# AlanLiangC/SPSNet

Measured on NVIDIA B200. Metric: IA-SSD SA-backbone scenes/s (16k pts), higher is better.
Workload: dtype fp16 operands / fp32 accumulate (split-fp16 hi+lo for K <= 64 chains and all Conv1d GEMMs); fp32 + int32 sampling

## Files before the change

spsnet_b200/csrc/pw_mma.cu:

```cuda
#include "mma_ptx.cuh"

namespace spsk {

constexpr int PW_ROWS = 128;
constexpr int PW_THREADS = 192;
constexpr int PW_TILE_BYTES = 16384;
constexpr int pw_smem(int stages, bool split) { return 256 + stages * (split ? 4 : 2) * PW_TILE_BYTES; }

struct PwArgs {
    int rows, k, ldx, n, npad, n_kc, relu;
    int split, xlo;
    int o16lo;
    const __half *x;
    const __half *wtiles;
    const float *bias;
    float *out_cm; int m, c_total, co_off;
    __half *out16; int ld16, n16;
    float *out_pm; int ldpm;
    unsigned int *ovf; unsigned int ovf_bit;
};

template <int PW_STAGES, int PW_LAG, bool SPLIT>
__global__ void __launch_bounds__(PW_THREADS, (PW_STAGES <= 3 && !SPLIT) ? 2 : 1)
pw_mma_kernel(const PwArgs a) {
    constexpr int STAGE_BYTES = (SPLIT ? 4 : 2) * PW_TILE_BYTES;
    extern __shared__ __align__(128) uint8_t smem[];
    uint64_t *bars = reinterpret_cast<uint64_t *>(smem);
    uint32_t *tmem_slot = reinterpret_cast<uint32_t *>(smem + 192);
    uint8_t *stage0 = smem + 256;
    const uint32_t bar0 = smem_u32(bars);
    auto FULL = [&](int s) { return bar0 + 8u * s; };
    auto EMPTY = [&](int s) { return bar0 + 8u * (PW_STAGES + s); };
    const uint32_t ACC_FULL = bar0 + 8u * (2 * PW_STAGES);
    auto XS = [&](int s) { return stage0 + (size_t)s * STAGE_BYTES; };
    auto WS = [&](int s) { return stage0 + (size_t)s * STAGE_BYTES + (SPLIT ? 2 : 1) * PW_TILE_BYTES; };

    const int tid = threadIdx.x, warp = tid >> 5, lane = tid & 31;
    const int tile = blockIdx.x, cc = blockIdx.y;
    const int ncols = min(128, a.npad - cc * 128);

    if (tid == 0) {
        for (int s = 0; s < PW_STAGES; ++s) { mbar_init(FULL(s), 128 + 1); mbar_init(EMPTY(s), 1); }
        mbar_init(ACC_FULL, 1);
        mbar_init_fence();
    }
    if (warp == 5) tmem_alloc(smem_u32(tmem_slot), 128);
    tc_fence_before();
    __syncthreads();
    tc_fence_after();
    const uint32_t tmem_base = *tmem_slot;

    if (warp == 4) {
        const bool leader = elect_one();
        for (int kc = 0; kc < a.n_kc; ++kc) {
            const int s = kc % PW_STAGES;
            const uint32_t ph = (kc / PW_STAGES) & 1u;
            mbar_wait(EMPTY(s), ph ^ 1u);
            if (leader) {
                constexpr uint32_t WB = (SPLIT ? 2 : 1) * PW_TILE_BYTES;
                mbar_expect_tx(FULL(s), WB);
                bulk_g2s(smem_u32(WS(s)), a.wtiles + (size_t)(cc * a.n_kc + kc) * (WB / 2), WB, FULL(s));
            }
            __syncwarp();
        }
    } else if (warp == 5) {
        const bool leader = elect_one();
        const uint32_t idesc = umma_idesc(128, ncols);
        for (int kc = 0; kc < a.n_kc; ++kc) {
            const int s = kc % PW_STAGES;
            const uint32_t ph = (kc / PW_STAGES) & 1u;
            mbar_wait(FULL(s), ph);
            tc_fence_after();
            const uint32_t xb = smem_u32(XS(s)), wb = smem_u32(WS(s));
            const int nk16 = min(4, (a.k - kc * 64) / 16);
            if (leader) {
                for (int j = 0; j < nk16; ++j) {
                    const uint64_t xh = umma_desc(xb + (uint32_t)j * 256u, 128u, 1024u), wh = umma_desc(wb + (uint32_t)j * 256u, 128u, 1024u);
                    umma_f16(tmem_base, xh, wh, idesc, (kc | j) ? 1u : 0u);
                    if (SPLIT) {
                        umma_f16(tmem_base, umma_desc(xb + PW_TILE_BYTES + (uint32_t)j * 256u, 128u, 1024u), wh, idesc, 1u);
                        umma_f16(tmem_base, xh, umma_desc(wb + PW_TILE_BYTES + (uint32_t)j * 256u, 128u, 1024u), idesc, 1u);
                    }
                }
                umma_commit(EMPTY(s));
                if (kc == a.n_kc - 1) umma_commit(ACC_FULL);
            }
            __syncwarp();
        }
    } else {
        const int r8 = lane & 7, gq = lane >> 3;
        for (int kc = 0; kc < a.n_kc; ++kc) {
            const int s = kc % PW_STAGES;
            const uint32_t ph = (kc / PW_STAGES) & 1u;
            mbar_wait(EMPTY(s), ph ^ 1u);
            const uint32_t xs = smem_u32(XS(s));
            const int ng = min(8, (a.k - kc * 64) / 8);
#pragma unroll
            for (int it = 0; it < 4; ++it) {
                const int r = warp * 32 + it * 8 + r8;
                const long long row = (long long)tile * PW_ROWS + r;
                const bool ok = row < a.rows;
                const __half *src = a.x + (size_t)(ok ? row : 0) * a.ldx;
#pragma unroll
                for (int j = 0; j < 2; ++j) {
                    const int g = gq + 4 * j;
                    if (g < ng) {
                        const int col = kc * 64 + g * 8;
                        const uint32_t dst = xs + (uint32_t)(r >> 3) * 1024u + (uint32_t)g * 128u + (uint32_t)(r & 7) * 16u;
                        cp_async16(dst, src + col, ok ? 16u : 0u);
                        if (SPLIT) cp_async16(dst + PW_TILE_BYTES, src + a.xlo + col, ok ? 16u : 0u);
                    }
                }
            }
            cp_async_commit();
            if (kc >= PW_LAG) {
                cp_async_wait<PW_LAG>();
                fence_proxy_async();
                mbar_arrive(FULL((kc - PW_LAG) % PW_STAGES));
            }
        }
        cp_async_wait<0>();
        fence_proxy_async();
        for (int kc = max(a.n_kc - PW_LAG, 0); kc < a.n_kc; ++kc) mbar_arrive(FULL(kc % PW_STAGES));

        mbar_wait(ACC_FULL, 0u);
        tc_fence_after();
        const int r = tid;
        const long long row = (long long)tile * PW_ROWS + r;
        const bool ok = row < a.rows;
        const uint32_t taddr = tmem_base + ((uint32_t)(warp * 32) << 16);
        const int ch0 = cc * 128;
        long long bb = 0;
        int p = 0;
        if (a.out_cm && ok) { bb = row / a.m; p = (int)(row - bb * a.m); }
        float mx16 = 0.f;
        for (int c0 = 0; c0 < ncols; c0 += 16) {
            float v[16];
            __syncwarp();
            tmem_ld16(taddr + (uint32_t)c0, v);
            const float4 *b4 = reinterpret_cast<const float4 *>(a.bias + ch0 + c0);
#pragma unroll
            for (int i = 0; i < 4; ++i) {
                const float4 bv = __ldg(b4 + i);
                v[4 * i] += bv.x; v[4 * i + 1] += bv.y; v[4 * i + 2] += bv.z; v[4 * i + 3] += bv.w;
            }
            if (a.relu) {
#pragma unroll
                for (int i = 0; i < 16; ++i) v[i] = fmaxf(v[i], 0.f);
            }
            if (ok && a.out_cm) {
                float *o = a.out_cm + ((size_t)bb * a.c_total + a.co_off + ch0 + c0) * a.m + p;
#pragma unroll
                for (int i = 0; i < 16; ++i)
                    if (ch0 + c0 + i < a.n) o[(size_t)i * a.m] = v[i];
            }
            if (ok && a.out16) {
                __half *o = a.out16 + (size_t)row * a.ld16 + ch0 + c0;
#pragma unroll
                for (int q = 0; q < 2; ++q)
                    if (ch0 + c0 + 8 * q < a.n16) {
                        uint32_t h[4], l[4];
#pragma unroll
                        for (int i = 0; i < 4; ++i) {
                            mx16 = fmaxf(fmaxf(mx16, fabsf(v[8 * q + 2 * i])), fabsf(v[8 * q + 2 * i + 1]));
                            const __half2 hh = __floats2half2_rn(v[8 * q + 2 * i], v[8 * q + 2 * i + 1]);
                            const float2 hf = __half22float2(hh);
                            h[i] = *reinterpret_cast<const uint32_t *>(&hh);
                            l[i] = pack_h2(v[8 * q + 2 * i] - hf.x, v[8 * q + 2 * i + 1] - hf.y);
                        }
                        *reinterpret_cast<uint4 *>(o + 8 * q) = make_uint4(h[0], h[1], h[2], h[3]);
                        if (a.o16lo > 0) *reinterpret_cast<uint4 *>(o + a.o16lo + 8 * q) = make_uint4(l[0], l[1], l[2], l[3]);
                    }
            }
            if (ok && a.out_pm) {
                float *o = a.out_pm + (size_t)row * a.ldpm + ch0 + c0;
#pragma unroll
                for (int i = 0; i < 16; ++i)
                    if (ch0 + c0 + i < a.n) o[i] = v[i];
            }
        }
        if (mx16 > FP16_MAX && a.ovf) atomicOr(a.ovf, a.ovf_bit);
    }

    tc_fence_before();
    __syncthreads();
    if (warp == 5) {
        tc_fence_after();
        tmem_dealloc(tmem_base, 128);
    }
}

}

extern "C" int spsk_pw_mma_forward(const spsk_pw_desc *d, spsk_stream_t stream) {
    using namespace spsk;
    SPSK_REQUIRE(d, SPSK_ERR_INVALID_ARG, "pw_mma: null descriptor");
    SPSK_REQUIRE(d->rows >= 0 && d->n >= 1 && d->k >= 16 && d->k % 16 == 0 && d->ldx >= d->k && d->ldx % 8 == 0, SPSK_ERR_INVALID_ARG,
                 "pw_mma: bad sizes rows=%d k=%d ldx=%d n=%d (k multiple of 16, ldx multiple of 8)", d->rows, d->k, d->ldx, d->n);
    if (d->rows == 0) return SPSK_OK;
    SPSK_REQUIRE(d->x && d->wtiles && d->bias, SPSK_ERR_INVALID_ARG, "pw_mma: null input pointer");
    SPSK_REQUIRE(d->out_cm || d->out16 || d->out_pm, SPSK_ERR_INVALID_ARG, "pw_mma: no output requested");
    SPSK_REQUIRE((reinterpret_cast<uintptr_t>(d->x) & 15) == 0 && (reinterpret_cast<uintptr_t>(d->wtiles) & 15) == 0, SPSK_ERR_INVALID_ARG,
                 "pw_mma: x / wtiles must be 16-byte aligned");
    PwArgs a{};
    a.rows = d->rows; a.k = d->k; a.ldx = d->ldx; a.n = d->n; a.relu = d->relu ? 1 : 0;
    a.npad = (d->n + 15) / 16 * 16;
    a.split = d->split ? 1 : 0;
    a.xlo = d->xlo;
    a.n_kc = (d->k + 63) / 64;
    if (a.split)
        SPSK_REQUIRE(d->xlo >= d->k && d->xlo % 8 == 0 && d->xlo + d->k <= d->ldx, SPSK_ERR_INVALID_ARG,
                     "pw_mma: split input needs the lo part at a column xlo >= k, multiple of 8, inside ldx");
    a.x = reinterpret_cast<const __half *>(d->x);
    a.wtiles = reinterpret_cast<const __half *>(d->wtiles);
    a.bias = d->bias;
    a.out_cm = d->out_cm; a.m = d->m; a.c_total = d->c_total; a.co_off = d->co_off;
    if (a.out_cm)
        SPSK_REQUIRE(d->m >= 1 && d->rows % d->m == 0 && d->co_off >= 0 && d->co_off + d->n <= d->c_total, SPSK_ERR_INVALID_ARG,
                     "pw_mma: channel-major output needs rows %% m == 0 and a channel window inside c_total");
    a.out16 = reinterpret_cast<__half *>(d->out16); a.ld16 = d->ld16; a.n16 = d->n16; a.o16lo = d->o16lo;
    if (a.out16 && d->o16lo)
        SPSK_REQUIRE(d->o16lo >= d->n16 && d->o16lo % 8 == 0 && d->o16lo + d->n16 <= d->ld16, SPSK_ERR_INVALID_ARG,
                     "pw_mma: residual columns [o16lo, o16lo + n16) must follow the values inside ld16");
    if (a.out16)
        SPSK_REQUIRE(d->ld16 % 8 == 0 && d->n16 % 8 == 0 && d->n16 >= d->n && d->n16 <= d->ld16 &&
                         (reinterpret_cast<uintptr_t>(d->out16) & 15) == 0,
                     SPSK_ERR_INVALID_ARG, "pw_mma: fp16 output needs ld16, n16 multiples of 8, n <= n16 <= ld16, 16-byte alignment");
    a.out_pm = d->out_pm; a.ldpm = d->ldpm;
    a.ovf = fp16_overflow_word();
    a.ovf_bit = 1u << (d->ovf_tag & 31);
    if (a.out_pm) SPSK_REQUIRE(d->ldpm >= d->n, SPSK_ERR_INVALID_ARG, "pw_mma: ldpm < n");
    const bool deep = !a.split && a.n_kc >= 12;
    static SmemAttrOnce attr_s, attr_d, attr_x;
    if (a.split) {
        if (int rc = attr_x.ensure(reinterpret_cast<const void *>(pw_mma_kernel<3, 2, true>), pw_smem(3, true), "pw_mma_kernel<3,2,split>")) return rc;
    } else if (deep) {
        if (int rc = attr_d.ensure(reinterpret_cast<const void *>(pw_mma_kernel<6, 4, false>), pw_smem(6, false), "pw_mma_kernel<6,4>")) return rc;
    } else {
        if (int rc = attr_s.ensure(reinterpret_cast<const void *>(pw_mma_kernel<3, 2, false>), pw_smem(3, false), "pw_mma_kernel<3,2>")) return rc;
    }
    const int ncover = a.out16 ? max(a.npad, a.n16) : a.npad;
    a.npad = (ncover + 15) / 16 * 16;
    dim3 grid((unsigned)((d->rows + PW_ROWS - 1) / PW_ROWS), (unsigned)((a.npad + 127) / 128));
    if (a.split) pw_mma_kernel<3, 2, true><<<grid, PW_THREADS, pw_smem(3, true), as_stream(stream)>>>(a);
    else if (deep) pw_mma_kernel<6, 4, false><<<grid, PW_THREADS, pw_smem(6, false), as_stream(stream)>>>(a);
    else pw_mma_kernel<3, 2, false><<<grid, PW_THREADS, pw_smem(3, false), as_stream(stream)>>>(a);
    SPSK_LAUNCH_CHECK("pw_mma_kernel");
    return SPSK_OK;
}
```

Baseline: 12010.

## Make pointwise MMA kernel persistent with double-buffered TMEM and column-tile grouping

Result: no change. 12010, median of 6 (-0.0%).

```diff
diff --git a/spsnet_b200/csrc/pw_mma.cu b/spsnet_b200/csrc/pw_mma.cu
--- a/spsnet_b200/csrc/pw_mma.cu
+++ b/spsnet_b200/csrc/pw_mma.cu
@@ -3,14 +3,22 @@
 namespace spsk {
 
 constexpr int PW_ROWS = 128;
-constexpr int PW_THREADS = 192;
+constexpr int PW_THREADS = 320;
 constexpr int PW_TILE_BYTES = 16384;
-constexpr int pw_smem(int stages, bool split) { return 256 + stages * (split ? 4 : 2) * PW_TILE_BYTES; }
+constexpr int PW_HDR = 256;
+constexpr int PW_MAX_STAGES = 8;
+constexpr int PW_SMEM_TWO = 113 * 1024;
+constexpr int PW_SMEM_MAX = 227 * 1024;
 
 struct PwArgs {
     int rows, k, ldx, n, npad, n_kc, relu;
     int split, xlo;
     int o16lo;
+    int stages, lag;
+    int nct, gtiles, ngroups;
+    int items;
+    int wbytes;
+    int acc_cols;
     const __half *x;
     const __half *wtiles;
     const float *bias;
@@ -20,173 +28,236 @@
     unsigned int *ovf; unsigned int ovf_bit;
 };
 
-template <int PW_STAGES, int PW_LAG, bool SPLIT>
-__global__ void __launch_bounds__(PW_THREADS, (PW_STAGES <= 3 && !SPLIT) ? 2 : 1)
+__device__ __forceinline__ void cp_async_wait_n(int n) {
+    switch (n) {
+        case 1: cp_async_wait<1>(); break;
+        case 2: cp_async_wait<2>(); break;
+        case 3: cp_async_wait<3>(); break;
+        default: cp_async_wait<4>(); break;
+    }
+}
+
+__device__ __forceinline__ void pw_wait(uint32_t bar, uint32_t parity) {
+#pragma unroll 1
+    for (uint32_t spin = 0; spin < (1u << 27); ++spin) {
+        uint32_t done;
+        asm volatile(
+            "{\n\t.reg .pred p;\n\t"
+            "mbarrier.test_wait.parity.shared::cta.b64 p, [%1], %2;\n\t"
+            "selp.b32 %0, 1, 0, p;\n\t}"
+            : "=r"(done)
+            : "r"(bar), "r"(parity)
+            : "memory");
+        if (done) return;
+    }
+    __trap();
+}
+
+template <bool SPLIT>
+__global__ void __launch_bounds__(PW_THREADS, 2)
 pw_mma_kernel(const PwArgs a) {
-    constexpr int STAGE_BYTES = (SPLIT ? 4 : 2) * PW_TILE_BYTES;
+    constexpr uint32_t XBYTES = (SPLIT ? 2 : 1) * PW_TILE_BYTES;
+    constexpr uint32_t WTBYTES = (SPLIT ? 2 : 1) * PW_TILE_BYTES;
     extern __shared__ __align__(128) uint8_t smem[];
-    uint64_t *bars = reinterpret_cast<uint64_t *>(smem);
-    uint32_t *tmem_slot = reinterpret_cast<uint32_t *>(smem + 192);
-    uint8_t *stage0 = smem + 256;
-    const uint32_t bar0 = smem_u32(bars);
+    uint32_t *tmem_slot = reinterpret_cast<uint32_t *>(smem + PW_HDR - 16);
+    const int S = a.stages;
+    const uint32_t stage_bytes = XBYTES + (uint32_t)a.wbytes;
+    const uint32_t bar0 = smem_u32(smem), ring = bar0 + PW_HDR;
     auto FULL = [&](int s) { return bar0 + 8u * s; };
-    auto EMPTY = [&](int s) { return bar0 + 8u * (PW_STAGES + s); };
-    const uint32_t ACC_FULL = bar0 + 8u * (2 * PW_STAGES);
-    auto XS = [&](int s) { return stage0 + (size_t)s * STAGE_BYTES; };
-    auto WS = [&](int s) { return stage0 + (size_t)s * STAGE_BYTES + (SPLIT ? 2 : 1) * PW_TILE_BYTES; };
+    auto EMPTY = [&](int s) { return bar0 + 8u * (S + s); };
+    auto ACC_FULL = [&](uint32_t b) { return bar0 + 8u * (2 * S + b); };
+    auto ACC_EMPTY = [&](uint32_t b) { return bar0 + 8u * (2 * S + 2 + b); };
+    auto XS = [&](int s) { return ring + (uint32_t)s * stage_bytes; };
+    auto WS = [&](int s) { return ring + (uint32_t)s * stage_bytes + XBYTES; };
+    auto NCOLS = [&](int cc) { return min(128, a.npad - cc * 128); };
 
     const int tid = threadIdx.x, warp = tid >> 5, lane = tid & 31;
-    const int tile = blockIdx.x, cc = blockIdx.y;
-    const int ncols = min(128, a.npad - cc * 128);
 
     if (tid == 0) {
-        for (int s = 0; s < PW_STAGES; ++s) { mbar_init(FULL(s), 128 + 1); mbar_init(EMPTY(s), 1); }
-        mbar_init(ACC_FULL, 1);
+        for (int s = 0; s < S; ++s) { mbar_init(FULL(s), 128 + 1); mbar_init(EMPTY(s), 1); }
+        for (uint32_t b = 0; b < 2; ++b) { mbar_init(ACC_FULL(b), 1); mbar_init(ACC_EMPTY(b), 128); }
         mbar_init_fence();
     }
-    if (warp == 5) tmem_alloc(smem_u32(tmem_slot), 128);
+    if (warp == 9) tmem_alloc(smem_u32(tmem_slot), 2u * (uint32_t)a.acc_cols);
     tc_fence_before();
     __syncthreads();
     tc_fence_after();
     const uint32_t tmem_base = *tmem_slot;
 
-    if (warp == 4) {
+    if (warp == 8) {
         const bool leader = elect_one();
-        for (int kc = 0; kc < a.n_kc; ++kc) {
-            const int s = kc % PW_STAGES;
-            const uint32_t ph = (kc / PW_STAGES) & 1u;
-            mbar_wait(EMPTY(s), ph ^ 1u);
-            if (leader) {
-                constexpr uint32_t WB = (SPLIT ? 2 : 1) * PW_TILE_BYTES;
-                mbar_expect_tx(FULL(s), WB);
-                bulk_g2s(smem_u32(WS(s)), a.wtiles + (size_t)(cc * a.n_kc + kc) * (WB / 2), WB, FULL(s));
+        uint32_t q = 0;
+        for (int item = blockIdx.x; item < a.items; item += gridDim.x) {
+            const int cc0 = (item % a.ngroups) * a.gtiles, nt = min(a.gtiles, a.nct - cc0);
+            for (int kc = 0; kc < a.n_kc; ++kc, ++q) {
+                const int s = (int)(q % (uint32_t)S);
+                pw_wait(EMPTY(s), ((q / (uint32_t)S) & 1u) ^ 1u);
+                if (leader) {
+                    mbar_expect_tx(FULL(s), (uint32_t)(min(a.npad - cc0 * 128, nt * 128) * 128 * (SPLIT ? 2 : 1)));
+                    for (int t = 0; t < nt; ++t) {
+                        const int cc = cc0 + t;
+                        const uint32_t wb = (uint32_t)NCOLS(cc) * 128u;
+                        const __half *src = a.wtiles + (size_t)(cc * a.n_kc + kc) * (WTBYTES / 2);
+                        const uint32_t dst = WS(s) + (uint32_t)t * WTBYTES;
+                        if (SPLIT && wb < (uint32_t)PW_TILE_BYTES) {
+                            bulk_g2s(dst, src, wb, FULL(s));
+                            bulk_g2s(dst + wb, src + PW_TILE_BYTES / 2, wb, FULL(s));
+                        } else {
+                            bulk_g2s(dst, src, SPLIT ? 2u * wb : wb, FULL(s));
+                        }
+                    }
+                }
+                __syncwarp();
             }
-            __syncwarp();
         }
-    } else if (warp == 5) {
+    } else if (warp == 9) {
         const bool leader = elect_one();
-        const uint32_t idesc = umma_idesc(128, ncols);
-        for (int kc = 0; kc < a.n_kc; ++kc) {
-            const int s = kc % PW_STAGES;
-            const uint32_t ph = (kc / PW_STAGES) & 1u;
-            mbar_wait(FULL(s), ph);
+        uint32_t q = 0, i = 0;
+        for (int item = blockIdx.x; item < a.items; item += gridDim.x, ++i) {
+            const int cc0 = (item % a.ngroups) * a.gtiles, nt = min(a.gtiles, a.nct - cc0);
+            const uint32_t acc = i & 1u;
+            pw_wait(ACC_EMPTY(acc), ((i >> 1) & 1u) ^ 1u);
             tc_fence_after();
-            const uint32_t xb = smem_u32(XS(s)), wb = smem_u32(WS(s));
-            const int nk16 = min(4, (a.k - kc * 64) / 16);
-            if (leader) {
-                for (int j = 0; j < nk16; ++j) {
-                    const uint64_t xh = umma_desc(xb + (uint32_t)j * 256u, 128u, 1024u), wh = umma_desc(wb + (uint32_t)j * 256u, 128u, 1024u);
-                    umma_f16(tmem_base, xh, wh, idesc, (kc | j) ? 1u : 0u);
-                    if (SPLIT) {
-                        umma_f16(tmem_base, umma_desc(xb + PW_TILE_BYTES + (uint32_t)j * 256u, 128u, 1024u), wh, idesc, 1u);
-                        umma_f16(tmem_base, xh, umma_desc(wb + PW_TILE_BYTES + (uint32_t)j * 256u, 128u, 1024u), idesc, 1u);
-                    }
-                }
-                umma_commit(EMPTY(s));
-                if (kc == a.n_kc - 1) umma_commit(ACC_FULL);
+            const uint32_t d0 = tmem_base + acc * (uint32_t)a.acc_cols;
+            for (int kc = 0; kc < a.n_kc; ++kc, ++q) {
+                const int s = (int)(q % (uint32_t)S);
+                pw_wait(FULL(s), (q / (uint32_t)S) & 1u);
+                tc_fence_after();
+                const uint32_t xb = XS(s), wb = WS(s);
+                const int nk16 = min(4, (a.k - kc * 64) / 16);
+                if (leader) {
+                    for (int j = 0; j < nk16; ++j) {
+                        const uint64_t xh = umma_desc(xb + (uint32_t)j * 256u, 128u, 1024u);
+                        for (int t = 0; t < nt; ++t) {
+                            const int nc = NCOLS(cc0 + t);
+                            const uint32_t idesc = umma_idesc(128, nc), d = d0 + (uint32_t)t * 128u;
+                            const uint32_t wt = wb + (uint32_t)t * WTBYTES + (uint32_t)j * 256u;
+                            const uint64_t wh = umma_desc(wt, 128u, 1024u);
+                            umma_f16(d, xh, wh, idesc, (kc | j) ? 1u : 0u);
+                            if (SPLIT) {
+                                umma_f16(d, umma_desc(xb + PW_TILE_BYTES + (uint32_t)j * 256u, 128u, 1024u), wh, idesc, 1u);
+                                umma_f16(d, xh, umma_desc(wt + (uint32_t)nc * 128u, 128u, 1024u), idesc, 1u);
+                            }
+                        }
+                    }
+                    umma_commit(EMPTY(s));
+                    if (kc == a.n_kc - 1) umma_commit(ACC_FULL(acc));
+                }
+                __syncwarp();
             }
-            __syncwarp();
         }
-    } else {
-        const int r8 = lane & 7, gq = lane >> 3;
-        for (int kc = 0; kc < a.n_kc; ++kc) {
-            const int s = kc % PW_STAGES;
-            const uint32_t ph = (kc / PW_STAGES) & 1u;
-            mbar_wait(EMPTY(s), ph ^ 1u);
-            const uint32_t xs = smem_u32(XS(s));
-            const int ng = min(8, (a.k - kc * 64) / 8);
-#pragma unroll
-            for (int it = 0; it < 4; ++it) {
-                const int r = warp * 32 + it * 8 + r8;
-                const long long row = (long long)tile * PW_ROWS + r;
-                const bool ok = row < a.rows;
-                const __half *src = a.x + (size_t)(ok ? row : 0) * a.ldx;
-#pragma unroll
-                for (int j = 0; j < 2; ++j) {
-                    const int g = gq + 4 * j;
-                    if (g < ng) {
-                        const int col = kc * 64 + g * 8;
-                        const uint32_t dst = xs + (uint32_t)(r >> 3) * 1024u + (uint32_t)g * 128u + (uint32_t)(r & 7) * 16u;
-                        cp_async16(dst, src + col, ok ? 16u : 0u);
-                        if (SPLIT) cp_async16(dst + PW_TILE_BYTES, src + a.xlo + col, ok ? 16u : 0u);
-                    }
-                }
-            }
-            cp_async_commit();
-            if (kc >= PW_LAG) {
-                cp_async_wait<PW_LAG>();
-                fence_proxy_async();
-                mbar_arrive(FULL((kc - PW_LAG) % PW_STAGES));
+    } else if (warp >= 4) {
+        const int r8 = lane & 7, gq = lane >> 3, lw = warp - 4;
+        uint32_t q = 0;
+        for (int item = blockIdx.x; item < a.items; item += gridDim.x) {
+            const long long row0 = (long long)(item / a.ngroups) * PW_ROWS;
+            for (int kc = 0; kc < a.n_kc; ++kc, ++q) {
+                const int s = (int)(q % (uint32_t)S);
+                pw_wait(EMPTY(s), ((q / (uint32_t)S) & 1u) ^ 1u);
+                const uint32_t xs = XS(s);
+                const int ng = min(8, (a.k - kc * 64) / 8);
+#pragma unroll
+                for (int it = 0; it < 4; ++it) {
+                    const int r = lw * 32 + it * 8 + r8;
+                    const long long row = row0 + r;
+                    const bool ok = row < a.rows;
+                    const __half *src = a.x + (size_t)(ok ? row : 0) * a.ldx;
+#pragma unroll
+                    for (int j = 0; j < 2; ++j) {
+                        const int g = gq + 4 * j;
+                        if (g < ng) {
+                            const int col = kc * 64 + g * 8;
+                            const uint32_t dst = xs + (uint32_t)(r >> 3) * 1024u + (uint32_t)g * 128u + (uint32_t)(r & 7) * 16u;
+                            cp_async16(dst, src + col, ok ? 16u : 0u);
+                            if (SPLIT) cp_async16(dst + PW_TILE_BYTES, src + a.xlo + col, ok ? 16u : 0u);
+                        }
+                    }
+                }
+                cp_async_commit();
+                if (q >= (uint32_t)a.lag) {
+                    cp_async_wait_n(a.lag);
+                    fence_proxy_async();
+                    mbar_arrive(FULL((int)((q - a.lag) % (uint32_t)S)));
+                }
             }
         }
         cp_async_wait<0>();
         fence_proxy_async();
-        for (int kc = max(a.n_kc - PW_LAG, 0); kc < a.n_kc; ++kc) mbar_arrive(FULL(kc % PW_STAGES));
-
-        mbar_wait(ACC_FULL, 0u);
-        tc_fence_after();
-        const int r = tid;
-        const long long row = (long long)tile * PW_ROWS + r;
-        const bool ok = row < a.rows;
-        const uint32_t taddr = tmem_base + ((uint32_t)(warp * 32) << 16);
-        const int ch0 = cc * 128;
-        long long bb = 0;
-        int p = 0;
-        if (a.out_cm && ok) { bb = row / a.m; p = (int)(row - bb * a.m); }
+        for (uint32_t p = q > (uint32_t)a.lag ? q - a.lag : 0u; p < q; ++p) mbar_arrive(FULL((int)(p % (uint32_t)S)));
+    } else {
+        const uint32_t lane_base = tmem_base + ((uint32_t)(warp * 32) << 16);
         float mx16 = 0.f;
-        for (int c0 = 0; c0 < ncols; c0 += 16) {
-            float v[16];
-            __syncwarp();
-            tmem_ld16(taddr + (uint32_t)c0, v);
-            const float4 *b4 = reinterpret_cast<const float4 *>(a.bias + ch0 + c0);
-#pragma unroll
-            for (int i = 0; i < 4; ++i) {
-                const float4 bv = __ldg(b4 + i);
-                v[4 * i] += bv.x; v[4 * i + 1] += bv.y; v[4 * i + 2] += bv.z; v[4 * i + 3] += bv.w;
+        uint32_t i = 0;
+        for (int item = blockIdx.x; item < a.items; item += gridDim.x, ++i) {
+            const int cc0 = (item % a.ngroups) * a.gtiles, nt = min(a.gtiles, a.nct - cc0);
+            const uint32_t acc = i & 1u;
+            pw_wait(ACC_FULL(acc), (i >> 1) & 1u);
+            tc_fence_after();
+            const long long row = (long long)(item / a.ngroups) * PW_ROWS + tid;
+            const bool ok = row < a.rows;
+            long long bb = 0;
+            int p = 0;
+            if (a.out_cm && ok) { bb = row / a.m; p = (int)(row - bb * a.m); }
+            for (int t = 0; t < nt; ++t) {
+                const int ch0 = (cc0 + t) * 128, ncols = NCOLS(cc0 + t);
+                const uint32_t taddr = lane_base + acc * (uint32_t)a.acc_cols + (uint32_t)t * 128u;
+                for (int c0 = 0; c0 < ncols; c0 += 16) {
+                    float v[16];
+                    __syncwarp();
+                    tmem_ld16(taddr + (uint32_t)c0, v);
+                    const float4 *b4 = reinterpret_cast<const float4 *>(a.bias + ch0 + c0);
+#pragma unroll
+                    for (int i4 = 0; i4 < 4; ++i4) {
+                        const float4 bv = __ldg(b4 + i4);
+                        v[4 * i4] += bv.x; v[4 * i4 + 1] += bv.y; v[4 * i4 + 2] += bv.z; v[4 * i4 + 3] += bv.w;
+                    }
+                    if (a.relu) {
+#pragma unroll
+                        for (int e = 0; e < 16; ++e) v[e] = fmaxf(v[e], 0.f);
+                    }
+                    if (ok && a.out_cm) {
+                        float *o = a.out_cm + ((size_t)bb * a.c_total + a.co_off + ch0 + c0) * a.m + p;
+#pragma unroll
+                        for (int e = 0; e < 16; ++e)
+                            if (ch0 + c0 + e < a.n) o[(size_t)e * a.m] = v[e];
+                    }
+                    if (ok && a.out16) {
+                        __half *o = a.out16 + (size_t)row * a.ld16 + ch0 + c0;
+#pragma unroll
+                        for (int h2 = 0; h2 < 2; ++h2)
+                            if (ch0 + c0 + 8 * h2 < a.n16) {
+                                uint32_t h[4], l[4];
+#pragma unroll
+                                for (int e = 0; e < 4; ++e) {
+                                    mx16 = fmaxf(fmaxf(mx16, fabsf(v[8 * h2 + 2 * e])), fabsf(v[8 * h2 + 2 * e + 1]));
+                                    const __half2 hh = __floats2half2_rn(v[8 * h2 + 2 * e], v[8 * h2 + 2 * e + 1]);
+                                    const float2 hf = __half22float2(hh);
+                                    h[e] = *reinterpret_cast<const uint32_t *>(&hh);
+                                    l[e] = pack_h2(v[8 * h2 + 2 * e] - hf.x, v[8 * h2 + 2 * e + 1] - hf.y);
+                                }
+                                *reinterpret_cast<uint4 *>(o + 8 * h2) = make_uint4(h[0], h[1], h[2], h[3]);
+                                if (a.o16lo > 0) *reinterpret_cast<uint4 *>(o + a.o16lo + 8 * h2) = make_uint4(l[0], l[1], l[2], l[3]);
+                            }
+                    }
+                    if (ok && a.out_pm) {
+                        float *o = a.out_pm + (size_t)row * a.ldpm + ch0 + c0;
+#pragma unroll
+                        for (int e = 0; e < 16; ++e)
+                            if (ch0 + c0 + e < a.n) o[e] = v[e];
+                    }
+                }
             }
-            if (a.relu) {
-#pragma unroll
-                for (int i = 0; i < 16; ++i) v[i] = fmaxf(v[i], 0.f);
-            }
-            if (ok && a.out_cm) {
-                float *o = a.out_cm + ((size_t)bb * a.c_total + a.co_off + ch0 + c0) * a.m + p;
-#pragma unroll
-                for (int i = 0; i < 16; ++i)
-                    if (ch0 + c0 + i < a.n) o[(size_t)i * a.m] = v[i];
-            }
-            if (ok && a.out16) {
-                __half *o = a.out16 + (size_t)row * a.ld16 + ch0 + c0;
-#pragma unroll
-                for (int q = 0; q < 2; ++q)
-                    if (ch0 + c0 + 8 * q < a.n16) {
-                        uint32_t h[4], l[4];
-#pragma unroll
-                        for (int i = 0; i < 4; ++i) {
-                            mx16 = fmaxf(fmaxf(mx16, fabsf(v[8 * q + 2 * i])), fabsf(v[8 * q + 2 * i + 1]));
-                            const __half2 hh = __floats2half2_rn(v[8 * q + 2 * i], v[8 * q + 2 * i + 1]);
-                            const float2 hf = __half22float2(hh);
-                            h[i] = *reinterpret_cast<const uint32_t *>(&hh);
-                            l[i] = pack_h2(v[8 * q + 2 * i] - hf.x, v[8 * q + 2 * i + 1] - hf.y);
-                        }
-                        *reinterpret_cast<uint4 *>(o + 8 * q) = make_uint4(h[0], h[1], h[2], h[3]);
-                        if (a.o16lo > 0) *reinterpret_cast<uint4 *>(o + a.o16lo + 8 * q) = make_uint4(l[0], l[1], l[2], l[3]);
-                    }
-            }
-            if (ok && a.out_pm) {
-                float *o = a.out_pm + (size_t)row * a.ldpm + ch0 + c0;
-#pragma unroll
-                for (int i = 0; i < 16; ++i)
-                    if (ch0 + c0 + i < a.n) o[i] = v[i];
-            }
+            tc_fence_before();
+            mbar_arrive(ACC_EMPTY(acc));
         }
         if (mx16 > FP16_MAX && a.ovf) atomicOr(a.ovf, a.ovf_bit);
     }
 
     tc_fence_before();
     __syncthreads();
-    if (warp == 5) {
+    if (warp == 9) {
         tc_fence_after();
-        tmem_dealloc(tmem_base, 128);
+        tmem_dealloc(tmem_base, 2u * (uint32_t)a.acc_cols);
     }
 }
 
@@ -230,21 +301,38 @@
     a.ovf = fp16_overflow_word();
     a.ovf_bit = 1u << (d->ovf_tag & 31);
     if (a.out_pm) SPSK_REQUIRE(d->ldpm >= d->n, SPSK_ERR_INVALID_ARG, "pw_mma: ldpm < n");
-    const bool deep = !a.split && a.n_kc >= 12;
-    static SmemAttrOnce attr_s, attr_d, attr_x;
-    if (a.split) {
-        if (int rc = attr_x.ensure(reinterpret_cast<const void *>(pw_mma_kernel<3, 2, true>), pw_smem(3, true), "pw_mma_kernel<3,2,split>")) return rc;
-    } else if (deep) {
-        if (int rc = attr_d.ensure(reinterpret_cast<const void *>(pw_mma_kernel<6, 4, false>), pw_smem(6, false), "pw_mma_kernel<6,4>")) return rc;
-    } else {
-        if (int rc = attr_s.ensure(reinterpret_cast<const void *>(pw_mma_kernel<3, 2, false>), pw_smem(3, false), "pw_mma_kernel<3,2>")) return rc;
-    }
     const int ncover = a.out16 ? max(a.npad, a.n16) : a.npad;
     a.npad = (ncover + 15) / 16 * 16;
-    dim3 grid((unsigned)((d->rows + PW_ROWS - 1) / PW_ROWS), (unsigned)((a.npad + 127) / 128));
-    if (a.split) pw_mma_kernel<3, 2, true><<<grid, PW_THREADS, pw_smem(3, true), as_stream(stream)>>>(a);
-    else if (deep) pw_mma_kernel<6, 4, false><<<grid, PW_THREADS, pw_smem(6, false), as_stream(stream)>>>(a);
-    else pw_mma_kernel<3, 2, false><<<grid, PW_THREADS, pw_smem(3, false), as_stream(stream)>>>(a);
+    a.nct = (a.npad + 127) / 128;
+
+    const int row_tiles = (d->rows + PW_ROWS - 1) / PW_ROWS;
+    a.gtiles = (a.nct >= 2 && (long long)row_tiles * ((a.nct + 1) / 2) >= SPSK_NUM_SMS) ? 2 : 1;
+    a.ngroups = (a.nct + a.gtiles - 1) / a.gtiles;
+    SPSK_REQUIRE((long long)row_tiles * a.ngroups <= 0x7FFFFFFF, SPSK_ERR_INVALID_ARG, "pw_mma: too many rows");
+    a.items = row_tiles * a.ngroups;
+    const int gcols = min(a.npad, a.gtiles * 128);
+    a.acc_cols = 32;
+    while (a.acc_cols < gcols) a.acc_cols *= 2;
+    a.wbytes = gcols * 128 * (a.split ? 2 : 1);
+
+    const int stage = (a.split ? 2 : 1) * PW_TILE_BYTES + a.wbytes;
+    int ctas = 1;
+    a.stages = (PW_SMEM_TWO - PW_HDR) / stage;
+    if (a.stages >= 2 && 2 * a.acc_cols <= 256) ctas = 2;
+    else a.stages = (PW_SMEM_MAX - PW_HDR) / stage;
+    a.stages = min(a.stages, PW_MAX_STAGES);
+    a.lag = min(a.stages - 1, 4);
+    const int smem = PW_HDR + a.stages * stage;
+    const int grid = min(a.items, SPSK_NUM_SMS * ctas);
+
+    static SmemAttrOnce attr_p, attr_x;
+    if (a.split) {
+        if (int rc = attr_x.ensure(reinterpret_cast<const void *>(pw_mma_kernel<true>), PW_SMEM_MAX, "pw_mma_kernel<split>")) return rc;
+        pw_mma_kernel<true><<<grid, PW_THREADS, smem, as_stream(stream)>>>(a);
+    } else {
+        if (int rc = attr_p.ensure(reinterpret_cast<const void *>(pw_mma_kernel<false>), PW_SMEM_MAX, "pw_mma_kernel")) return rc;
+        pw_mma_kernel<false><<<grid, PW_THREADS, smem, as_stream(stream)>>>(a);
+    }
     SPSK_LAUNCH_CHECK("pw_mma_kernel");
     return SPSK_OK;
 }
```
